# SEU-dynamical-models/Manifold-based-optical-flow-method

Measured on AMD Instinct MI355X. Metric: flow timesteps/sec on 160k-vertex mesh, higher is better.
Workload: dtype f32

## Files before the change

manifold-based-optical-flow-method_amd/csrc/mof_amg.hip:

```cpp
#include <algorithm>
#include <cstdio>
#include <cstdlib>

#include "mof_amg.h"
#include "mof_rowkern.h"

int mof_io_guard(const std::function<void()> &f);

namespace mof {

std::atomic<int> g_force_galerkin_ns{0};
enum GalKernel { kGal0Ns, kGal0Ent, kGalSys2F32, kGalSys2Bf16, kGalSys3, kGal3Ns, kGal3Ent, kGal3Big, kGalKernels };
std::atomic<int64_t> g_galerkin_launches[kGalKernels];

namespace {

constexpr int kB3 = 12;

__device__ __forceinline__ bool retired(const int32_t *sysi, int32_t b) {
    return !sysi[b * kSysStride + SI_ACTIVE] || sysi[b * kSysStride + SI_CONV] >= 0;
}

template <int BS>
__device__ __forceinline__ void ldv(const float *v, int64_t node, float (&x)[BS]) {
// ... 1063 lines not shown
        const int32_t i = F.rent[2 * (int64_t)e];
        const float *p = F.Q + (int64_t)F.rent[2 * (int64_t)e + 1] * (BSF * 3);
        float pm[BSF * 3];
#pragma unroll
        for (int k = 0; k < BSF * 3; ++k) pm[k] = p[k];
        float ri[kNSR][BSF];
#pragma unroll
        for (int t = 0; t < kNSR; ++t) ldr<BSF>(F.r, sm_b(F.sm, b0 + t), F.n, i, ri[t]);
#pragma unroll
        for (int t = 0; t < kNSR; ++t)
#pragma unroll
            for (int c = 0; c < 3; ++c) {
                float v = pm[c] * ri[t][0] + pm[3 + c] * ri[t][1];
                if constexpr (BSF == 3) v += pm[6 + c] * ri[t][2];
                c3[t][c] = v;
            }
    };
    for (int32_t q = e0 + threadIdx.x; q < e1 && !big; q += 2 * kWG) {
        const bool two = q + kWG < e1;
        const int32_t ea = F.rperm ? F.rperm[q] : q;
        const int32_t eb = two ? (F.rperm ? F.rperm[q + kWG] : q + kWG) : ea;
        float c3[2][kNSR][3];
        contrib(ea, c3[0]);
        contrib(eb, c3[1]);
#pragma unroll
        for (int t = 0; t < kNSR; ++t)
#pragma unroll
            for (int c = 0; c < 3; ++c) con[t][c][ea - e0] = c3[0][t][c];
        if (two)
#pragma unroll
            for (int t = 0; t < kNSR; ++t)
#pragma unroll
                for (int c = 0; c < 3; ++c) con[t][c][eb - e0] = c3[1][t][c];
    }
    __syncthreads();
    const int32_t nI = I1 - I0;
    for (int32_t q = threadIdx.x; q < nI * kNSR; q += kWG) {
        const int32_t t = q / nI, I = I0 + q - t * nI;
        if (b0 + t >= F.sm.n) continue;
        const int32_t b = sm_b(F.sm, b0 + t);
        if (retired(sysi, b)) continue;
        float acc[3] = {};
        for (int32_t e = F.rptr[I]; e < F.rptr[I + 1]; ++e) {
            float c3[3];
            if (big) {
                float all[kNSR][3];
                contrib(e, all);
#pragma unroll
                for (int c = 0; c < 3; ++c) c3[c] = all[t][c];
            } else {
#pragma unroll
                for (int c = 0; c < 3; ++c) c3[c] = con[t][c][e - e0];
            }
#pragma unroll
            for (int c = 0; c < 3; ++c) acc[c] += c3[c];
        }
        const int64_t vo = (int64_t)b * C.n * 4;
        stv<3>(C.b + vo, I, acc);
        if (smooth) {
            float d[3][3], x[3];
            ld_dh(C, b, I, d);
            matvec<3>(d, acc, x);
#pragma unroll
            for (int c = 0; c < 3; ++c) x[c] *= omega;
            stv<3>(C.x + vo, I, x);
        }
    }
}

template <int XM>
__global__ __launch_bounds__(kWG) void k_prolong0_sa(Lvl F, Lvl C, int32_t nblk, int32_t B,
                                                     const int32_t *__restrict__ sysi) {
#pragma clang fp contract(off)
    int32_t rb, bq;
    const int32_t nq = (F.sm.n + kNSP - 1) / kNSP;
    if (!xcd_map(nblk, nq, rb, bq, kGrpProl)) return;
    const int32_t b0 = bq * kNSP;
    const int32_t i = rb * kWG + threadIdx.x;
    if (i >= F.n) return;
    float x[kNSP][2];
#pragma unroll
    for (int t = 0; t < kNSP; ++t) {
        const float2 v = ld_x0(F.x, (int64_t)sm_b(F.sm, b0 + t) * F.n + i);
        x[t][0] = v.x;
        x[t][1] = v.y;
    }
    const int32_t k0 = F.pptr[i], k1 = F.pptr[i + 1];
    for (int32_t k = k0; k < k1; ++k) {
        const int32_t K = F.pcol[k];
        const float *q = F.Q + (int64_t)k * 6;
        float qm[6];
#pragma unroll
        for (int c = 0; c < 6; ++c) qm[c] = q[c];
        float y[kNSP][3];
#pragma unroll
        for (int t = 0; t < kNSP; ++t) ldv<3>(C.y + (int64_t)sm_b(F.sm, b0 + t) * C.n * 4, K, y[t]);
#pragma unroll
        for (int t = 0; t < kNSP; ++t) {
            x[t][0] += qm[0] * y[t][0] + qm[1] * y[t][1] + qm[2] * y[t][2];
            x[t][1] += qm[3] * y[t][0] + qm[4] * y[t][1] + qm[5] * y[t][2];
        }
    }
#pragma unroll
    for (int t = 0; t < kNSP; ++t) {
        if (b0 + t >= F.sm.n) continue;
        const int32_t b = sm_b(F.sm, b0 + t);
        if (retired(sysi, b)) continue;
        if constexpr (XM == 2)
            reinterpret_cast<float2 *>(F.y)[(int64_t)b * F.n + i] = make_float2(x[t][0], x[t][1]);
        else
            st_x0(F.x, (int64_t)b * F.n + i, x[t][0], x[t][1]);
    }
}

constexpr int kNS3 = 8;
__global__ __launch_bounds__(kWG) void k_prolong3_sa(Lvl F, Lvl C, int32_t nblk, int32_t B,
                                                     const int32_t *__restrict__ sysi) {
#pragma clang fp contract(off)
    int32_t rb, bq;
    if (!xcd_map(nblk, (F.sm.n + kNS3 - 1) / kNS3, rb, bq, kGrpProl)) return;
    const int32_t i = rb * kWG + threadIdx.x;
    if (i >= F.n) return;
    const int32_t b0 = bq * kNS3;
    float x[kNS3][3];
#pragma unroll
    for (int t = 0; t < kNS3; ++t) ldv<3>(F.x + (int64_t)sm_b(F.sm, b0 + t) * F.n * 4, i, x[t]);
    for (int32_t k = F.pptr[i]; k < F.pptr[i + 1]; ++k) {
        const float *p = F.Q + (int64_t)k * 9;
        float pm[9];
#pragma unroll
        for (int c = 0; c < 9; ++c) pm[c] = p[c];
        const int32_t K = F.pcol[k];
        float y[kNS3][3];
#pragma unroll
        for (int t = 0; t < kNS3; ++t) ldv<3>(C.y + (int64_t)sm_b(F.sm, b0 + t) * C.n * 4, K, y[t]);
#pragma unroll
        for (int t = 0; t < kNS3; ++t)
#pragma unroll
            for (int r = 0; r < 3; ++r) x[t][r] += pm[3 * r] * y[t][0] + pm[3 * r + 1] * y[t][1] + pm[3 * r + 2] * y[t][2];
    }
#pragma unroll
    for (int t = 0; t < kNS3; ++t) {
        if (b0 + t >= F.sm.n) continue;
        const int32_t b = sm_b(F.sm, b0 + t);
        if (retired(sysi, b)) continue;
        stv<3>(F.x + (int64_t)b * F.n * 4, i, x[t]);
    }
}

template <int BSF>
__global__ __launch_bounds__(kWG) void k_prolong(Lvl F, Lvl C, const int32_t *__restrict__ sysi) {
    const int32_t i = blockIdx.x * kWG + threadIdx.x, b = sm_b(F.sm, blockIdx.y);
    if (i >= F.n || retired(sysi, b)) return;
    prolong_node<BSF>(F, C, b, i);
}

constexpr int kProlR = 1, kProlS = 4;
template <int XM>
__global__ __launch_bounds__(kWG) void k_prolong0(Lvl F, Lvl C, int32_t nblk, int32_t B,
                                                  const int32_t *__restrict__ sysi) {
#pragma clang fp contract(off)
    int32_t rb, bq;
    if (!xcd_map(nblk, (F.sm.n + kProlS - 1) / kProlS, rb, bq, kGrpProl)) return;
    const int32_t n = F.n;
    int32_t ii[kProlR], ag[kProlR];
    float q[kProlR][6];
#pragma unroll
    for (int r = 0; r < kProlR; ++r) {
        ii[r] = (rb * kProlR + r) * kWG + threadIdx.x;
        const int32_t i = min(ii[r], n - 1);
        ag[r] = F.agg[i];
#pragma unroll
        for (int k = 0; k < 6; ++k) q[r][k] = F.Q[(int64_t)i * 6 + k];
    }
    float2 x0[kProlS][kProlR];
    float y[kProlS][kProlR][3];
#pragma unroll
    for (int t = 0; t < kProlS; ++t) {
        const int32_t b = sm_b(F.sm, bq * kProlS + t);
        const float *yb = C.y + (int64_t)b * C.n * 4;
#pragma unroll
        for (int r = 0; r < kProlR; ++r) {
            x0[t][r] = ld_x0(F.x, (int64_t)b * n + min(ii[r], n - 1));
            ldv<3>(yb, ag[r], y[t][r]);
        }
    }
#pragma unroll
    for (int t = 0; t < kProlS; ++t) {
        if (bq * kProlS + t >= F.sm.n) continue;
        const int32_t b = sm_b(F.sm, bq * kProlS + t);
        if (retired(sysi, b)) continue;
        const int64_t vb = (int64_t)b * n;
#pragma unroll
        for (int r = 0; r < kProlR; ++r) {
            if (ii[r] >= n) break;
            float xi[2] = {x0[t][r].x, x0[t][r].y};
#pragma unroll
            for (int k = 0; k < 2; ++k)
                xi[k] += q[r][3 * k] * y[t][r][0] + q[r][3 * k + 1] * y[t][r][1] + q[r][3 * k + 2] * y[t][r][2];
            if constexpr (XM == 2)
                reinterpret_cast<float2 *>(F.y)[vb + ii[r]] = make_float2(xi[0], xi[1]);
            else
                st_x0(F.x, vb + ii[r], xi[0], xi[1]);
        }
    }
}

__global__ __launch_bounds__(kWG) void k_post3(Lvl L, float omega, const int32_t *__restrict__ sysi) {
    const int32_t i = blockIdx.x * kWG + threadIdx.x, b = sm_b(L.sm, blockIdx.y);
    if (i >= L.n || retired(sysi, b)) return;
    post3_node(L, b, i, omega);
}

constexpr int kSubWG = 512;
constexpr int kMaxLevels = 12;

struct SubArgs {
    int32_t first, last;
    Lvl lv[kMaxLevels];
    const float *cinv;
    float omega;
    const int32_t *sysi;
};

__global__ __launch_bounds__(kSubWG) void k_subcycle(SubArgs a) {
    const int32_t b = sm_b(a.lv[0].sm, blockIdx.x);
    if (retired(a.sysi, b)) return;
    const int32_t tid = threadIdx.x;
    for (int32_t l = a.first; l < a.last; ++l) {
        const Lvl &F = a.lv[l], &C = a.lv[l + 1];
        for (int32_t i = tid; i < F.n; i += kSubWG) res3_node(F, b, i);
        __syncthreads();
        for (int32_t I = tid; I < C.n; I += kSubWG) restrict_node<3>(F, C, b, I, l + 1 < a.last, a.omega);
        __syncthreads();
    }
    {
        constexpr int kH = kSubWG / kMaxCoarse;
        __shared__ float bl[kMaxCoarse];
        __shared__ float part[kH][kMaxCoarse];
        const Lvl &C = a.lv[a.last];
        const int32_t nc = 3 * C.n;
        const float *Mi = a.cinv + (int64_t)b * nc * nc;
        const float *bb = C.b + (int64_t)b * C.n * 4;
        for (int32_t q = tid; q < nc; q += kSubWG) bl[q] = bb[4 * (q / 3) + q % 3];
        __syncthreads();
        const int32_t d = tid % kMaxCoarse, hf = tid / kMaxCoarse;
        const int32_t chunk = (nc + kH - 1) / kH;
        const int32_t k0 = min(nc, hf * chunk), k1 = min(nc, k0 + chunk);
        float sum = 0.f;
        if (d < nc) {
            constexpr int U = 16;
            for (int32_t k = k0; k < k1; k += U) {
                float mv[U];
#pragma unroll
                for (int u = 0; u < U; ++u) mv[u] = Mi[(int64_t)min(k + u, k1 - 1) * nc + d];
#pragma unroll
                for (int u = 0; u < U; ++u) sum += (k + u < k1) ? mv[u] * bl[min(k + u, k1 - 1)] : 0.f;
            }
        }
        part[hf][d] = sum;
        __syncthreads();
        if (!hf && d < nc) {
            float t = part[0][d];
#pragma unroll
            for (int h = 1; h < kH; ++h) t += part[h][d];
            C.y[(int64_t)b * C.n * 4 + 4 * (d / 3) + d % 3] = t;
        }
        __syncthreads();
    }
    for (int32_t l = a.last - 1; l >= a.first; --l) {
        const Lvl &F = a.lv[l], &C = a.lv[l + 1];
        for (int32_t i = tid; i < F.n; i += kSubWG) prolong_node<3>(F, C, b, i);
        __syncthreads();
        for (int32_t i = tid; i < F.n; i += kSubWG) post3_node(F, b, i, a.omega);
        __syncthreads();
    }
}

constexpr int kRes0NS = 2, kRes0U = kSweepU;
template <int NS, bool PK>
__global__ __launch_bounds__(kWG) MOF_ROW_OCC void k_res0_ns(int32_t N, int32_t nblk, int32_t B, SysMap sm, MatH mat,
                                                 const float *__restrict__ rv, const float *__restrict__ xv,
                                                 const int32_t *__restrict__ apos,
                                                 const int32_t *__restrict__ sysi, float *__restrict__ r1) {
#pragma clang fp contract(off)
    int32_t rb, bq;
    if (!xcd_map(nblk, (sm.n + NS - 1) / NS, rb, bq, kGrpSmooth > NS ? kGrpSmooth / NS : 1)) return;
    int32_t bs[NS];
    bool act[NS];
    bool any = false;
#pragma unroll
    for (int t = 0; t < NS; ++t) {
        const int32_t l = bq * NS + t;
        bs[t] = sm_b(sm, l);
        act[t] = l < sm.n && !retired(sysi, bs[t]);
        any |= act[t];
    }
    if (!any) return;
#pragma unroll
    for (int r = 0; r < kRows; ++r) {
        const int32_t i = rb * kRowsPerWG + r * kWG + threadIdx.x;
        if (i >= N) break;
        float y[NS][2];
        auto xl = [&](int t, int32_t j) { return ld_x0(xv, (int64_t)bs[t] * N + j); };
        if constexpr (PK)
            spmv_row_hx_ns<kIxPack, NS, kRes0U>(mat, bs, i, xl, y);
        else if (mat.sell_mir)
            spmv_row_hx_ns<kIxMir, NS, kRes0U>(mat, bs, i, xl, y);
        else
            spmv_row_hx_ns<kIxPlain, NS, kRes0U>(mat, bs, i, xl, y);
#pragma unroll
        for (int t = 0; t < NS; ++t) {
            if (!act[t]) continue;
            const int64_t vb = (int64_t)bs[t] * N;
            const float2 ri = reinterpret_cast<const float2 *>(rv)[vb + i];
            reinterpret_cast<uint32_t *>(r1)[vb + (apos ? apos[i] : i)] =
                bf16_bits(ri.x - y[t][0]) | (bf16_bits(ri.y - y[t][1]) << 16);
        }
    }
}

constexpr int kPost0NS = 2, kPost0U = 4;
template <int XM, bool ZH, int NS, bool PK>
__global__ __launch_bounds__(kWG) MOF_ROW_OCC void k_post0_ns(int32_t N, int32_t nblk, int32_t B, SysMap sm, MatH mat,
                                                  const float *__restrict__ rv,
                                                  const float *__restrict__ xv, float omega,
                                                  const int32_t *__restrict__ sysi,
                                                  float *__restrict__ zv, double *__restrict__ part,
                                                  RedArgs rd) {
#pragma clang fp contract(off)
    __shared__ double lds[8 * NS];
    int32_t rb, bq;
    if (!xcd_map(nblk, (sm.n + NS - 1) / NS, rb, bq, kGrpSmooth > NS ? kGrpSmooth / NS : 1)) return;
    int32_t bs[NS];
    bool act[NS];
    bool any = false;
#pragma unroll
    for (int t = 0; t < NS; ++t) {
        const int32_t l = bq * NS + t;
        bs[t] = sm_b(sm, l);
        act[t] = l < sm.n && !retired(sysi, bs[t]);
        any |= act[t];
    }
    if (!any) return;
    double rz[NS];
#pragma unroll
    for (int t = 0; t < NS; ++t) rz[t] = 0.0;
#pragma unroll
    for (int g = 0; g < kRows; ++g) {
        const int32_t i = rb * kRowsPerWG + g * kWG + threadIdx.x;
        if (i >= N) break;
        float y[NS][2];
        uint2 dg[NS];
        auto xl = [&](int t, int32_t j) {
            const int64_t vj = (int64_t)bs[t] * N + j;
            if constexpr (XM == 2)
                return reinterpret_cast<const float2 *>(xv)[vj];
            else
                return ld_x0(xv, vj);
        };
        if constexpr (PK)
            spmv_row_hx_ns<kIxPack, NS, kPost0U>(mat, bs, i, xl, y, dg);
        else if (mat.sell_mir)
            spmv_row_hx_ns<kIxMir, NS, kPost0U>(mat, bs, i, xl, y, dg);
        else
            spmv_row_hx_ns<kIxPlain, NS, kPost0U>(mat, bs, i, xl, y, dg);
#pragma unroll
        for (int t = 0; t < NS; ++t) {
            const int64_t vb = (int64_t)bs[t] * N;
            const float2 xi = xl(t, i);
            const float2 ri = reinterpret_cast<const float2 *>(rv)[vb + i];
            const float2 ds = bf16_diag_solve(dg[t], ri.x - y[t][0], ri.y - y[t][1]);
            float z0 = xi.x + omega * ds.x;
            float z1 = xi.y + omega * ds.y;
            if constexpr (ZH) {
                const uint32_t h = bf16_bits(z0) | (bf16_bits(z1) << 16);
                if (act[t]) reinterpret_cast<uint32_t *>(zv)[vb + i] = h;
                z0 = bf16_lo(h);
                z1 = bf16_hi(h);
            } else {
                if (act[t]) reinterpret_cast<float2 *>(zv)[vb + i] = make_float2(z0, z1);
            }
            if (i < rd.nown) rz[t] += (double)ri.x * z0 + (double)ri.y * z1;
        }
    }
    block_sum<NS>(rz, lds);
    if (threadIdx.x == 0) {
#pragma unroll
        for (int t = 0; t < NS; ++t)
            if (act[t]) part[2 * (((int64_t)rd.part * B + bs[t]) * rd.nmax + rb)] = rz[t];
    }
}

constexpr int kBswWG = 1024;
constexpr int32_t kBswOff = INT32_MIN;
constexpr int64_t kBswLdsMax = 160 * 1024;
struct BswArgs {
    int32_t N, nbr, nout, nslot;
    const int32_t *rows, *roff, *wrow, *xsrc, *ocol;
    const uint2 *A;
};
template <bool F32X>
__device__ __forceinline__ float2 bsw_ldx(const float *xv, int64_t vj) {
    if constexpr (F32X)
        return reinterpret_cast<const float2 *>(xv)[vj];
    else
        return ld_x0(xv, vj);
}
__global__ __launch_bounds__(kWG) void k_bsw_extract(int32_t nslot, int32_t B, const int32_t *__restrict__ bsrc,
                                                     const uint2 *__restrict__ A0h, int64_t sell_nb,
                                                     uint2 *__restrict__ out) {
    const int64_t q = (int64_t)blockIdx.x * kWG + threadIdx.x;
    if (q >= (int64_t)nslot * B) return;
    const int32_t b = (int32_t)(q / nslot), t = (int32_t)(q - (int64_t)b * nslot);
    const int32_t src = bsrc[t];
    uint2 h = make_uint2(0u, 0u);
    if (src >= 0) {
        h = h0_ld(A0h, (int64_t)b * sell_nb + (src & kMirPos));
        if (src & kMirT) h = h0_tr(h);
    }
    out[q] = h;
}
template <bool F32X>
__global__ __launch_bounds__(kBswWG) void k_bsweep(BswArgs a, SysMap sm, const float *__restrict__ rv,
                                                   float *__restrict__ xv, float omega, int32_t sweeps,
                                                   const int32_t *__restrict__ sysi) {
#pragma clang fp contract(off)
    extern __shared__ float2 bsw_lds[];
    if ((int32_t)blockIdx.x >= sm.n) return;
    const int32_t b = sm_b(sm, blockIdx.x);
    if (retired(sysi, b)) return;
    const int64_t vb = (int64_t)b * a.N;
    float2 *xs[2] = {bsw_lds, bsw_lds + a.nbr};
    float2 *xo = bsw_lds + 2 * a.nbr;
    for (int32_t p = threadIdx.x; p < a.nbr; p += kBswWG) xs[0][p] = bsw_ldx<F32X>(xv, vb + a.rows[p]);
    for (int32_t k = threadIdx.x; k < a.nout; k += kBswWG) xo[k] = bsw_ldx<F32X>(xv, vb + a.ocol[k]);
    __syncthreads();
    const uint2 *Ab = a.A + (int64_t)b * a.nslot;
    constexpr int U = kPost0U;
    int cur = 0;
    for (int32_t k = 0; k < sweeps; ++k) {
        for (int32_t p = threadIdx.x; p < a.nbr; p += kBswWG) {
            const int32_t base = a.roff[p >> 6] + (p & 63), w = a.wrow[p];
            const float2 ri = reinterpret_cast<const float2 *>(rv)[vb + a.rows[p]];
            float acc0 = 0.f, acc1 = 0.f;
            uint2 dg = make_uint2(0u, 0u);
            for (int32_t t0 = 0; t0 < w; t0 += U) {
                int32_t src[U];
                uint2 blk[U];
#pragma unroll
                for (int u = 0; u < U; ++u) {
                    const int32_t q = base + min(t0 + u, w - 1) * kSlice;
                    src[u] = a.xsrc[q];
                    blk[u] = Ab[q];
                }
                if (t0 == 0) dg = blk[0];
#pragma unroll
                for (int u = 0; u < U; ++u) {
                    const bool on = t0 + u < w && src[u] != kBswOff;
                    float2 xj = make_float2(0.f, 0.f);
                    if (on) xj = src[u] >= 0 ? xs[cur][src[u]] : xo[-1 - src[u]];
                    float e00, e01, e10, e11;
                    h0_dec(blk[u], e00, e01, e10, e11);
                    acc0 += on ? e00 * xj.x + e01 * xj.y : 0.f;
                    acc1 += on ? e10 * xj.x + e11 * xj.y : 0.f;
                }
            }
            const float2 ds = bf16_diag_solve(dg, ri.x - acc0, ri.y - acc1);
            const float2 xi = xs[cur][p];
            xs[cur ^ 1][p] = make_float2(xi.x + omega * ds.x, xi.y + omega * ds.y);
        }
        __syncthreads();
        cur ^= 1;
    }
    for (int32_t p = threadIdx.x; p < a.nbr; p += kBswWG) {
        const float2 v = xs[cur][p];
        if constexpr (F32X)
            reinterpret_cast<float2 *>(xv)[vb + a.rows[p]] = v;
        else
            st_x0(xv, vb + a.rows[p], v.x, v.y);
    }
}
BswArgs bsw_args(const AmgDevice &G) {
    BswArgs a;
    a.N = G.bsw_N;
    a.nbr = G.bsw_n;
    a.nout = G.bsw_nout;
    a.nslot = G.bsw_nslot;
    a.rows = G.bsw_rows.p;
    a.roff = G.bsw_roff.p;
    a.wrow = G.bsw_wrow.p;
    a.xsrc = G.bsw_xsrc.p;
    a.ocol = G.bsw_ocol.p;
    a.A = reinterpret_cast<const uint2 *>(G.bsw_A.p);
    return a;
}
template <bool F32X>
void launch_bsweep(const AmgDevice &G, SysMap sm, const float *rv, float *xv, float omega, const int32_t *sysi,
                   hipStream_t s) {
    const size_t lds = sizeof(float2) * (2 * (size_t)G.bsw_n + G.bsw_nout);
    k_bsweep<F32X><<<dim3((unsigned)sm.n), kBswWG, lds, s>>>(bsw_args(G), sm, rv, xv, omega, G.bsw_sweeps, sysi);
}

template <int XM, bool ZH, typename... Args>
void launch_post0(bool packed, int32_t nblk, int32_t B, hipStream_t s, Args... args) {
    const dim3 g(xcd_grid(nblk, (B + kPost0NS - 1) / kPost0NS, kGrpSmooth > kPost0NS ? kGrpSmooth / kPost0NS : 1));
    if (packed)
        k_post0_ns<XM, ZH, kPost0NS, true><<<g, kWG, 0, s>>>(args...);
    else
        k_post0_ns<XM, ZH, kPost0NS, false><<<g, kWG, 0, s>>>(args...);
}

inline dim3 grid2(int64_t n, int32_t B) { return dim3((unsigned)((n + kWG - 1) / kWG), (unsigned)B); }

MatH level0_mat(mof_mesh *m) {
    MatH mt;
    mt.sell_nb = m->pat.sell_nb();
    mt.sell_off = m->sell_off.p;
    mt.sell_col = m->sell_col.p;
    mt.sell_mir = m->sym_reads ? m->sell_mir.p : nullptr;
    mt.sell_idx = m->sym_reads && m->idx_packed ? m->sell_idx.p : nullptr;
    mt.vptr = m->sym_reads ? nullptr : m->vptr.p;
    mt.A = reinterpret_cast<const uint2 *>(m->amg->A0h.p);
    return mt;
}

}


bool amg_build(mof_mesh *m) {
    AmgParams prm;
    const bool open_surface = [&] {
        const int64_t E = ((int64_t)m->pat.nblocks() - m->N) / 2;
        return m->n_own == m->N && 3 * (int64_t)m->M != 2 * E;
    }();
    if (open_surface) {
        prm.omega = 0.7f;
        prm.smooth = 1;
    }
    float omega1_set = 0.f;
    if (const char *v = knob(Knob::AmgOmega)) {
        char *end = nullptr;
        prm.omega = std::strtof(v, &end);
        if (end && *end == ',') omega1_set = prm.omega1 = std::strtof(end + 1, nullptr);
    }
    if (knob(Knob::AmgSmooth)) prm.smooth = knob_int(Knob::AmgSmooth, 0) != 0;
    prm.smooth1 = -1;
    if (m->n_own < m->N) prm.nown = m->n_own;
    if (m->amg && m->amg->built) return m->amg->lv.size() >= 2;
    if (!m->amg) m->amg = new AmgDevice();
    AmgDevice &G = *m->amg;
    hipStream_t s = m->stream;
    MeshShared *sh = m->shared.get();
    char key[160];
    std::snprintf(key, sizeof(key), "%a/%a/%d/%d/%a/%d/%d", (double)prm.omega, (double)prm.omega1, prm.smooth,
                  prm.nown, (double)prm.smooth_omega, (int)m->sym_reads, prm.smooth1);
    std::unique_lock<std::mutex> build_lock;
    std::shared_ptr<const AmgHierarchy> Hp;
    if (sh) {
        build_lock = std::unique_lock<std::mutex>(sh->amg_build_mu);
        std::lock_guard<std::mutex> lk(sh->mu);
        for (const auto &kv : sh->amg)
            if (kv.first == key) Hp = kv.second;
    }
    if (!Hp) {
        std::vector<double> e(6 * (size_t)m->N);
        MOF_HIP(hipMemcpyAsync(e.data(), m->e.p, e.size() * sizeof(double), hipMemcpyDeviceToHost, s));
        MOF_HIP(hipStreamSynchronize(s));
        std::vector<double> a2;
        if (prm.nown < 0 && ((prm.smooth != 0 && (prm.smooth > 0 || amg_auto_smooth(m->pat))) || prm.smooth1 != 0)) {
            a2.resize(4 * (size_t)m->pat.sell_nb());
            MOF_HIP(hipMemcpyAsync(a2.data(), m->a2.p, a2.size() * sizeof(double), hipMemcpyDeviceToHost, s));
            MOF_HIP(hipStreamSynchronize(s));
            prm.a2 = a2.data();
        }
        if (!m->agg_order.empty()) prm.order = m->agg_order.data();
        const std::vector<int32_t> mir = sell_mirror(m->pat, m->n_own, 1, nullptr);
        prm.mirror = mir.data();
        auto built = std::make_shared<AmgHierarchy>();
        AmgParams p1 = prm;
        const bool l0_smooth = prm.nown < 0 && prm.a2 && prm.smooth != 0 && (prm.smooth > 0 || amg_auto_smooth(m->pat));
        p1.smooth1 = prm.smooth1 > 0 ? prm.smooth1 : (prm.smooth1 < 0 && l0_smooth ? 1 : 0);
        if (open_surface && p1.smooth1 == 1) p1.smooth1 = 2;
        build_amg(m->pat, e.data(), p1, *built);
        if (prm.smooth1 < 0 && p1.smooth1 == 0 && prm.nown < 0 && prm.a2 && !built->levels.empty() &&
            !built->levels[0].smoothed && built->max_curl >= kFoldCurl) {
            const double curl = built->max_curl;
            p1.smooth1 = 1;
            if (prm.smooth != 0 && !built->curl.empty() && built->curl[0] < kFlatCurl) p1.smooth = 1;
            auto again = std::make_shared<AmgHierarchy>();
            build_amg(m->pat, e.data(), p1, *again);
            again->max_curl = curl;
            again->folded = true;
            built = again;
        }
        built->mirror = mir;
        Hp = built;
        if (sh) {
            std::lock_guard<std::mutex> lk(sh->mu);
            sh->amg.emplace_back(key, Hp);
        }
    }
    if (build_lock.owns_lock()) build_lock.unlock();
    const AmgHierarchy &H = *Hp;
    G.H = Hp;
    G.omega = prm.omega;
    G.omega1 = prm.omega1;
    G.xm = 2;
    G.lv.clear();
    G.built = true;
    if (H.levels.size() < 2) return false;
    G.regular = !amg_auto_smooth(m->pat) && !open_surface;
    G.xm = G.regular ? 1 : 2;
    if (omega1_set <= 0.f) G.omega1 = G.regular ? 1.1f : 1.05f;
    MOF_REQUIRE(H.coarse_dofs <= kMaxCoarse, "coarsest multigrid level too large");
    MOF_REQUIRE(H.levels.size() <= (size_t)kMaxLevels, "too many multigrid levels");
    G.lv.resize(H.levels.size());
    auto put_i = [&](DevArray<int32_t> &d, const std::vector<int32_t> &h) {
        d.alloc(h.size());
        if (!h.empty()) d.upload(h.data(), h.size(), s);
    };
    auto put_f = [&](DevArray<float> &d, const std::vector<float> &h) {
        d.alloc(h.size());
        if (!h.empty()) d.upload(h.data(), h.size(), s);
    };
    G.bsw_n = 0;
    G.bsw_sweeps = 0;
    int32_t bsw = -1;
    if (knob(Knob::AmgBsw)) bsw = std::max(0, std::min(8, knob_int(Knob::AmgBsw, 0)));
    if (open_surface && bsw != 0) {
        const Pattern &P = m->pat;
        std::vector<uint8_t> mark(m->N, 0);
        for (int32_t i = 0; i < m->N; ++i) {
            const int32_t a = P.vptr[i], e2 = P.vptr[i + 1];
            const int32_t d = (int32_t)(std::lower_bound(P.vcol.begin() + a, P.vcol.begin() + e2, i) - P.vcol.begin());
            if (P.cptr[d + 1] - P.cptr[d] < e2 - a - 1) mark[i] = 1;
        }
        std::vector<uint8_t> ring(mark);
        for (int32_t i = 0; i < m->N; ++i)
            if (mark[i])
                for (int32_t q = P.vptr[i]; q < P.vptr[i + 1]; ++q) ring[P.vcol[q]] = 1;
        std::vector<int32_t> rows, pos(m->N, -1);
        for (int32_t i = 0; i < m->N; ++i)
            if (ring[i]) {
                pos[i] = (int32_t)rows.size();
                rows.push_back(i);
            }
        if (!rows.empty()) {
            const int32_t nbr = (int32_t)rows.size(), nrs = (nbr + kSlice - 1) / kSlice;
            std::vector<int32_t> mir;
            if (m->sym_reads) mir = sell_mirror(P, m->n_own, 1, nullptr);
            std::vector<int32_t> wrow(nbr), roff(nrs + 1, 0), ocol, opos(m->N, -1);
            for (int32_t p = 0; p < nbr; ++p) {
                const int32_t s0 = rows[p] / kSlice;
                wrow[p] = (int32_t)((P.sell_off[s0 + 1] - P.sell_off[s0]) / kSlice);
            }
            for (int32_t r = 0; r < nrs; ++r) {
                int32_t wmax = 0;
                for (int32_t p = r * kSlice; p < std::min(nbr, (r + 1) * kSlice); ++p) wmax = std::max(wmax, wrow[p]);
                roff[r + 1] = roff[r] + wmax * kSlice;
            }
            const int32_t nslot = roff[nrs];
            std::vector<int32_t> xsrc(nslot, kBswOff), bsrc(nslot, -1);
            for (int32_t p = 0; p < nbr; ++p) {
                const int32_t i = rows[p], s0 = i / kSlice, l = i % kSlice;
                const int64_t o = P.sell_off[s0];
                const int32_t w = wrow[p];
                const int32_t wl = m->sym_reads ? w : std::min(w, P.vptr[i + 1] - P.vptr[i]);
                for (int32_t t = 0; t < w; ++t) {
                    const int64_t pp = o + (int64_t)std::min(t, wl - 1) * kSlice + l;
                    const int32_t j = P.sell_col[pp];
                    int32_t src = (int32_t)pp;
                    bool on = t < wl;
                    if (m->sym_reads) {
                        const int32_t mr = mir[pp];
                        on = on && mr >= 0;
                        src = mr < 0 ? (int32_t)(o + l) : mr;
                    }
                    if (!on) continue;
                    const int64_t q = roff[p / kSlice] + (int64_t)t * kSlice + p % kSlice;
                    bsrc[q] = src;
                    if (pos[j] >= 0) {
                        xsrc[q] = pos[j];
                    } else {
                        if (opos[j] < 0) {
                            opos[j] = (int32_t)ocol.size();
                            ocol.push_back(j);
                        }
                        xsrc[q] = -1 - opos[j];
                    }
                }
            }
            const int64_t lds = (int64_t)sizeof(float2) * (2 * (int64_t)nbr + (int64_t)ocol.size());
            if (lds > kBswLdsMax) {
                if (knob(Knob::Verbose))
                    std::fprintf(stderr, "mof amg: boundary ring of %d rows needs %lld B of LDS: no boundary sweeps\n",
                                 nbr, (long long)lds);
            } else {
                put_i(G.bsw_rows, rows);
                put_i(G.bsw_roff, roff);
                put_i(G.bsw_wrow, wrow);
                put_i(G.bsw_xsrc, xsrc);
                put_i(G.bsw_bsrc, bsrc);
                put_i(G.bsw_ocol, ocol);
                G.bsw_N = m->N;
                G.bsw_n = nbr;
                G.bsw_nout = (int32_t)ocol.size();
                G.bsw_nslot = nslot;
                G.bsw_sweeps = bsw > 0 ? bsw : 2;
                if (knob(Knob::Verbose))
                    std::fprintf(stderr, "mof amg: boundary sweeps x%d on a ring of %d rows (%d outside, %lld B of LDS)\n",
                                 G.bsw_sweeps, nbr, G.bsw_nout, (long long)lds);
                static LdsLimit limit;
                raise_lds_limit(limit, m->device,
                                {reinterpret_cast<const void *>(&k_bsweep<true>),
                                 reinterpret_cast<const void *>(&k_bsweep<false>)},
                                kBswLdsMax);
            }
        }
    }
    for (size_t l = 0; l < H.levels.size(); ++l) {
        const AmgLevel &L = H.levels[l];
        AmgDevLevel &D = G.lv[l];
        D.n = L.n;
        D.bs = L.bs;
        D.sell_nb = L.sell_nb();
        if (l > 0) {
            {
                std::vector<int32_t> tw((size_t)L.sell_nb(), -1);
                for (size_t k = 0; k < L.low.size(); ++k) tw[L.twin[k]] = L.low[k];
                put_i(D.twin, tw);
            }
            put_i(D.sell_off, L.sell_off);
            put_i(D.sell_col, L.sell_col);
            put_i(D.sell_row, L.sell_row);
            put_i(D.diag_pos, L.diag_pos);
            D.dead.alloc(L.dead.size());
            D.dead.upload(L.dead.data(), L.dead.size(), s);
        }
        if (l + 1 < H.levels.size()) {
            put_i(D.agg, L.agg);
            put_i(D.mptr, L.mptr);
// ... 529 lines not shown
```

manifold-based-optical-flow-method_amd/csrc/mof_rowkern.h:

```cpp
#pragma once

#include "mof_internal.h"

namespace mof {
namespace {

template <typename V>
struct VT;
template <>
struct VT<float> {
    using V2 = float2;
};
template <>
struct VT<double> {
    using V2 = double2;
};

constexpr int kRows = 1;
constexpr int kRowsPerWG = kWG * kRows;

__device__ __forceinline__ void ld_blk(const float *A, int64_t pos, float (&a)[4]) {
    const float4 v = reinterpret_cast<const float4 *>(A)[pos];
    a[0] = v.x; a[1] = v.y; a[2] = v.z; a[3] = v.w;
}
__device__ __forceinline__ void ld_blk(const double *A, int64_t pos, double (&a)[4]) {
    const double2 v0 = reinterpret_cast<const double2 *>(A)[2 * pos];
    const double2 v1 = reinterpret_cast<const double2 *>(A)[2 * pos + 1];
    a[0] = v0.x; a[1] = v0.y; a[2] = v1.x; a[3] = v1.y;
}

__device__ __forceinline__ uint32_t bf16_bits(float f) {
    const uint32_t u = __float_as_uint(f);
    return (u + 0x7FFFu + ((u >> 16) & 1u)) >> 16;
}
__device__ __forceinline__ float bf16_lo(uint32_t w) { return __uint_as_float(w << 16); }
__device__ __forceinline__ float bf16_hi(uint32_t w) { return __uint_as_float(w & 0xFFFF0000u); }
__device__ __forceinline__ uint2 bf16x4(float a, float b, float c, float d) {
    return make_uint2(bf16_bits(a) | (bf16_bits(b) << 16), bf16_bits(c) | (bf16_bits(d) << 16));
}

__device__ __forceinline__ uint2 h0_ld(const uint2 *H, int64_t q) { return H[q]; }
__device__ __forceinline__ void h0_st(uint2 *H, int64_t q, float a, float b, float c, float d) {
    H[q] = bf16x4(a, b, c, d);
}
__device__ __forceinline__ uint2 h0_tr(uint2 h) {
    return make_uint2((h.x & 0xFFFFu) | (h.y << 16), (h.x >> 16) | (h.y & 0xFFFF0000u));
}
__device__ __forceinline__ void h0_dec(uint2 h, float &a00, float &a01, float &a10, float &a11) {
    a00 = bf16_lo(h.x); a01 = bf16_hi(h.x); a10 = bf16_lo(h.y); a11 = bf16_hi(h.y);
}

__device__ __forceinline__ double wave_sum(double v) {
#pragma unroll
    for (int o = 32; o > 0; o >>= 1) v += __shfl_down(v, o, 64);
    return v;
}

template <int NV, int NT = kWG>
__device__ __forceinline__ void block_sum(double (&v)[NV], double *lds) {
#pragma unroll
    for (int k = 0; k < NV; ++k) v[k] = wave_sum(v[k]);
    const int w = threadIdx.x >> 6;
    if ((threadIdx.x & 63) == 0) {
#pragma unroll
        for (int k = 0; k < NV; ++k) lds[w * NV + k] = v[k];
    }
    __syncthreads();
#pragma unroll
    for (int k = 0; k < NV; ++k) {
        double s = ((lds[k] + lds[NV + k]) + lds[2 * NV + k]) + lds[3 * NV + k];
#pragma unroll
        for (int q = 4; q < NT / 64; ++q) s += lds[q * NV + k];
        v[k] = s;
    }
    __syncthreads();
}

template <int NV, int NQ>
__device__ __forceinline__ void block_sum_q(double (&v)[NV], double *lds) {
    if constexpr (NQ == 1) {
        block_sum<NV, kWG>(v, lds);
    } else {
#pragma unroll
        for (int k = 0; k < NV; ++k) v[k] = wave_sum(v[k]);
        const int w = threadIdx.x >> 6;
        if ((threadIdx.x & 63) == 0) {
#pragma unroll
            for (int k = 0; k < NV; ++k) lds[w * NV + k] = v[k];
        }
        __syncthreads();
        const double *L = lds + (w & ~3) * NV;
#pragma unroll
        for (int k = 0; k < NV; ++k) v[k] = ((L[k] + L[NV + k]) + L[2 * NV + k]) + L[3 * NV + k];
        __syncthreads();
    }
}
__device__ __forceinline__ int32_t row_tid() { return (int32_t)(threadIdx.x & (kWG - 1)); }

__device__ __forceinline__ double wave_max(double v) {
#pragma unroll
    for (int o = 32; o > 0; o >>= 1) v = fmax(v, __shfl_down(v, o, 64));
    return v;
}
template <int NV, int NQ>
__device__ __forceinline__ void block_max_q(double (&v)[NV], double *lds) {
#pragma unroll
    for (int k = 0; k < NV; ++k) v[k] = wave_max(v[k]);
    const int w = threadIdx.x >> 6;
    if ((threadIdx.x & 63) == 0) {
#pragma unroll
        for (int k = 0; k < NV; ++k) lds[w * NV + k] = v[k];
    }
    __syncthreads();
    const double *L = lds + (w & ~3) * NV;
#pragma unroll
    for (int k = 0; k < NV; ++k) v[k] = fmax(fmax(L[k], L[NV + k]), fmax(L[2 * NV + k], L[3 * NV + k]));
    __syncthreads();
}
template <int NV, int NT>
__device__ __forceinline__ void block_max(double (&v)[NV], double *lds) {
#pragma unroll
    for (int k = 0; k < NV; ++k) v[k] = wave_max(v[k]);
    const int w = threadIdx.x >> 6;
    if ((threadIdx.x & 63) == 0) {
#pragma unroll
        for (int k = 0; k < NV; ++k) lds[w * NV + k] = v[k];
    }
    __syncthreads();
#pragma unroll
    for (int k = 0; k < NV; ++k) {
        double s = lds[k];
#pragma unroll
        for (int q = 1; q < NT / 64; ++q) s = fmax(s, lds[q * NV + k]);
        v[k] = s;
    }
    __syncthreads();
}

template <int NV, int NT = kWG>
__device__ __forceinline__ void reduce_partials(const double *part, int n, double (&out)[NV],
                                                double *lds) {
#pragma unroll
    for (int k = 0; k < NV; ++k) out[k] = 0.0;
    int q = threadIdx.x < kWG ? (int)threadIdx.x : n;
    for (; q + 3 * kWG < n; q += 4 * kWG) {
        double v[4][NV];
#pragma unroll
        for (int u = 0; u < 4; ++u)
#pragma unroll
            for (int k = 0; k < NV; ++k) v[u][k] = part[(int64_t)(q + u * kWG) * NV + k];
#pragma unroll
        for (int u = 0; u < 4; ++u)
#pragma unroll
            for (int k = 0; k < NV; ++k) out[k] += v[u][k];
    }
    for (; q < n; q += kWG) {
#pragma unroll
        for (int k = 0; k < NV; ++k) out[k] += part[(int64_t)q * NV + k];
    }
    block_sum<NV, NT>(out, lds);
}

template <typename V>
struct MatArgs {
    int64_t sell_nb;
    const int32_t *sell_off, *sell_col;
    const int32_t *sell_mir;
    const uint32_t *sell_idx;
    const int32_t *vptr;
    const V *A;
};

__device__ __forceinline__ int32_t row_width(const int32_t *vptr, int32_t i, int32_t w) {
    return vptr ? min(w, vptr[i + 1] - vptr[i]) : w;
}

__device__ __forceinline__ int64_t mir_pos(int32_t m, int64_t diag) { return m < 0 ? diag : (int64_t)(m & kMirPos); }

template <typename V>
__device__ __forceinline__ typename VT<V>::V2 ld2(const V *p) {
    return *reinterpret_cast<const typename VT<V>::V2 *>(p);
}

constexpr int kIxPlain = 0, kIxMir = 1, kIxPack = 2;
__device__ __forceinline__ int32_t idx_dcol(uint32_t w) { return (int32_t)(w << 16) >> 16; }
__device__ __forceinline__ int32_t idx_dpos(uint32_t w) { return (int32_t)w >> 16; }

__device__ __forceinline__ int32_t wave_slice(int32_t i) { return __builtin_amdgcn_readfirstlane(i >> 6); }

template <typename T>
__device__ __forceinline__ const T *byte_off(const T *base, uint32_t bytes) {
    return reinterpret_cast<const T *>(reinterpret_cast<const char *>(base) + bytes);
}
__device__ __forceinline__ void ld_blk32(const float *A, uint32_t pos, float (&a)[4]) {
    const float4 v = *byte_off(reinterpret_cast<const float4 *>(A), pos * 16u);
    a[0] = v.x; a[1] = v.y; a[2] = v.z; a[3] = v.w;
}
__device__ __forceinline__ void ld_blk32(const double *A, uint32_t pos, double (&a)[4]) { ld_blk(A, (int64_t)pos, a); }

#define MOF_ROW_OCC __attribute__((amdgpu_waves_per_eu(5, 8)))
constexpr int kSpmvU = 8, kSweepU = 8;

template <int IX, typename V, bool ZH = false>
__device__ __forceinline__ void spmv_row_t(const MatArgs<V> &mt, int32_t b, int32_t i,
                                           const V *__restrict__ x, V &y0, V &y1) {
#pragma clang fp contract(off)
    using V2 = typename VT<V>::V2;
    constexpr int U = kSpmvU;
    constexpr bool sym = IX != kIxPlain;
    const V *A = mt.A + 4 * (int64_t)b * mt.sell_nb;
    const int32_t s = wave_slice(i), l = i & 63;
    const int32_t o = mt.sell_off[s];
    const int32_t w = (mt.sell_off[s + 1] - o) >> 6;
    const int32_t wl = sym ? w : row_width(mt.vptr, i, w);
    V a0 = 0, a1 = 0;
    for (int32_t t0 = 0; t0 < w; t0 += U) {
        int32_t j[U], mr[U];
        V blk[U][4];
        V2 xj[U];
#pragma unroll
        for (int u = 0; u < U; ++u) {
            const int32_t t = min(t0 + u, wl - 1);
            if constexpr (IX == kIxPack) {
                const uint32_t iw = *byte_off(mt.sell_idx, (uint32_t)(o + t * kSlice + l) * 4u);
                j[u] = i + idx_dcol(iw);
                mr[u] = idx_dpos(iw);
            } else {
                j[u] = mt.sell_col[(int64_t)o + t * kSlice + l];
                if constexpr (sym) mr[u] = mt.sell_mir[(int64_t)o + t * kSlice + l];
            }
        }
#pragma unroll
        for (int u = 0; u < U; ++u) {
            const int32_t t = min(t0 + u, wl - 1);
            if constexpr (IX == kIxPack)
                ld_blk32(A, (uint32_t)(mr[u] == kIdxPad ? o + l : o + t * kSlice + l + mr[u]), blk[u]);
            else if constexpr (sym)
                ld_blk(A, mir_pos(mr[u], (int64_t)o + l), blk[u]);
            else
                ld_blk(A, (int64_t)o + t * kSlice + l, blk[u]);
        }
#pragma unroll
        for (int u = 0; u < U; ++u) {
            if constexpr (ZH) {
                const uint32_t h = reinterpret_cast<const uint32_t *>(x)[j[u]];
                xj[u] = V2{bf16_lo(h), bf16_hi(h)};
            } else {
                xj[u] = ld2(x + 2 * (int64_t)j[u]);
            }
        }
#pragma unroll
        for (int u = 0; u < U; ++u) {
            if constexpr (sym) {
                bool on, tr;
                if constexpr (IX == kIxPack) {
                    on = t0 + u < w && mr[u] != kIdxPad;
                    tr = mr[u] != 0;
                } else {
                    on = t0 + u < w && mr[u] >= 0;
                    tr = (mr[u] & kMirT) != 0;
                }
                const V b1 = tr ? blk[u][2] : blk[u][1], b2 = tr ? blk[u][1] : blk[u][2];
                a0 += on ? blk[u][0] * xj[u].x + b1 * xj[u].y : (V)0;
                a1 += on ? b2 * xj[u].x + blk[u][3] * xj[u].y : (V)0;
            } else {
                const bool on = t0 + u < wl;
                a0 += on ? blk[u][0] * xj[u].x + blk[u][1] * xj[u].y : (V)0;
                a1 += on ? blk[u][2] * xj[u].x + blk[u][3] * xj[u].y : (V)0;
            }
        }
    }
    y0 = a0;
    y1 = a1;
}
template <typename V, bool ZH = false>
__device__ __forceinline__ void spmv_row(const MatArgs<V> &mt, int32_t b, int32_t i,
                                         const V *__restrict__ x, V &y0, V &y1) {
    if (mt.sell_mir)
        spmv_row_t<kIxMir, V, ZH>(mt, b, i, x, y0, y1);
    else
        spmv_row_t<kIxPlain, V, ZH>(mt, b, i, x, y0, y1);
}

constexpr int32_t kGrpSpmv = 8, kGrpSmooth = 8, kGrpRes = 8, kGrpGal = 8, kGrpAsm = 8, kGrpProl = 8,
                  kGrpRestr = 8;
__host__ __device__ __forceinline__ int32_t sys_group(int32_t B, int32_t G) { return G > 0 && G < B ? G : B; }

__host__ __device__ __forceinline__ bool xcd_map_w(int32_t w, int32_t nblk, int32_t B, int32_t &rb, int32_t &sys,
                                                   int32_t grp_sz) {
    const int32_t q = w >> 3;
    const int32_t chunk = (nblk + 7) >> 3;
    const int32_t G = sys_group(B, grp_sz);
    const int32_t grp = q / (chunk * G), rem = q - grp * chunk * G;
    sys = grp * G + rem % G;
    rb = (w & 7) * chunk + rem / G;
    return rb < nblk && sys < B;
}
__device__ __forceinline__ bool xcd_map(int32_t nblk, int32_t B, int32_t &rb, int32_t &sys, int32_t grp_sz) {
    return xcd_map_w((int32_t)blockIdx.x, nblk, B, rb, sys, grp_sz);
}

inline unsigned xcd_grid(int32_t nblk, int32_t B, int32_t grp_sz) {
    const int64_t G = sys_group(B, grp_sz);
    const int64_t n = 8 * G * ((B + G - 1) / G) * ((nblk + 7) / 8);
    MOF_REQUIRE(n * kWG < ((int64_t)1 << 32), "launch grid past 2^32 work-items (batch too large for this mesh)");
    return (unsigned)n;
}
inline int32_t xcd_batch_cap(int64_t nblk, int32_t grp_sz) {
    const int64_t lim = (((int64_t)1 << 32) - 1) / kWG;
    const int64_t per = 8 * ((nblk + 7) / 8);
    int64_t B = std::min<int64_t>(lim / per, 1 << 30);
    auto n = [&](int64_t b) {
        const int64_t G = b > grp_sz && grp_sz > 0 ? grp_sz : b;
        return 8 * G * ((b + G - 1) / G) * ((nblk + 7) / 8);
    };
    while (B > 1 && n(B) > lim) --B;
    return (int32_t)std::max<int64_t>(1, B);
}


struct SysMap {
    const int32_t *map;
    int32_t n;
};
inline SysMap sys_all(int32_t B) { return SysMap{nullptr, B}; }
__device__ __forceinline__ int32_t sm_b(const SysMap &s, int32_t l) {
    l = min(l, s.n - 1);
    return s.map ? s.map[l] : l;
}

struct MatH {
    int64_t sell_nb;
    const int32_t *sell_off, *sell_col;
    const int32_t *sell_mir;
    const uint32_t *sell_idx;
    const int32_t *vptr;
    const uint2 *A;
};

template <int IX, int NS, int U = kSweepU, typename XL>
__device__ __forceinline__ void spmv_row_hx_ns(const MatH &mt, const int32_t (&bs)[NS], int32_t i, XL &&xload,
                                               float (&y)[NS][2], uint2 *diag = nullptr) {
#pragma clang fp contract(off)
    constexpr bool sym = IX != kIxPlain;
    using Pos = std::conditional_t<IX == kIxPack, uint32_t, int64_t>;
    const int32_t s = wave_slice(i), l = i & 63;
    const int32_t o = mt.sell_off[s];
    const int32_t w = (mt.sell_off[s + 1] - o) >> 6;
    const int32_t wl = sym ? w : row_width(mt.vptr, i, w);
    float acc[NS][2];
#pragma unroll
    for (int t = 0; t < NS; ++t) acc[t][0] = acc[t][1] = 0.f;
    for (int32_t t0 = 0; t0 < w; t0 += U) {
        int32_t j[U], mr[U];
        Pos pos[U];
#pragma unroll
        for (int u = 0; u < U; ++u) {
            if constexpr (IX == kIxPack) {
                const int32_t own = o + min(t0 + u, wl - 1) * kSlice + l;
                const uint32_t iw = *byte_off(mt.sell_idx, (uint32_t)own * 4u);
                j[u] = i + idx_dcol(iw);
                mr[u] = idx_dpos(iw);
                pos[u] = (uint32_t)(mr[u] == kIdxPad ? o + l : own + mr[u]);
            } else {
                pos[u] = (int64_t)o + min(t0 + u, wl - 1) * kSlice + l;
                j[u] = mt.sell_col[pos[u]];
                if constexpr (sym) mr[u] = mt.sell_mir[pos[u]];
            }
        }
        if constexpr (IX == kIxMir) {
#pragma unroll
            for (int u = 0; u < U; ++u) pos[u] = mir_pos(mr[u], (int64_t)o + l);
        }
        uint2 blk[NS][U];
        float2 xj[NS][U];
#pragma unroll
        for (int t = 0; t < NS; ++t) {
            if constexpr (IX == kIxPack) {
                const uint2 *Ab = mt.A + (int64_t)bs[t] * mt.sell_nb;
#pragma unroll
                for (int u = 0; u < U; ++u) blk[t][u] = *byte_off(Ab, pos[u] * 8u);
            } else {
#pragma unroll
                for (int u = 0; u < U; ++u) blk[t][u] = h0_ld(mt.A, (int64_t)bs[t] * mt.sell_nb + pos[u]);
            }
        }
        if (diag && t0 == 0) {
#pragma unroll
            for (int t = 0; t < NS; ++t) diag[t] = blk[t][0];
        }
#pragma unroll
        for (int t = 0; t < NS; ++t)
#pragma unroll
            for (int u = 0; u < U; ++u) xj[t][u] = xload(t, j[u]);
#pragma unroll
        for (int u = 0; u < U; ++u) {
            bool on = t0 + u < wl;
            bool tr = false;
            if constexpr (IX == kIxPack) {
                on = on && mr[u] != kIdxPad;
                tr = mr[u] != 0;
            } else if constexpr (sym) {
                on = on && mr[u] >= 0;
                tr = (mr[u] & kMirT) != 0;
            }
#pragma unroll
            for (int t = 0; t < NS; ++t) {
                const uint2 h = tr ? h0_tr(blk[t][u]) : blk[t][u];
                float e00, e01, e10, e11;
                h0_dec(h, e00, e01, e10, e11);
                acc[t][0] += on ? e00 * xj[t][u].x + e01 * xj[t][u].y : 0.f;
                acc[t][1] += on ? e10 * xj[t][u].x + e11 * xj[t][u].y : 0.f;
            }
        }
    }
#pragma unroll
    for (int t = 0; t < NS; ++t) {
        y[t][0] = acc[t][0];
        y[t][1] = acc[t][1];
    }
}

__device__ __forceinline__ float2 ld_x0(const float *x, int64_t vi) {
    const uint32_t h = reinterpret_cast<const uint32_t *>(x)[vi];
    return make_float2(bf16_lo(h), bf16_hi(h));
}
__device__ __forceinline__ void st_x0(float *x, int64_t vi, float a, float b) {
    reinterpret_cast<uint32_t *>(x)[vi] = bf16_bits(a) | (bf16_bits(b) << 16);
}

__device__ __forceinline__ float2 bf16_mat2(uint2 d, float v0, float v1) {
    return make_float2(bf16_lo(d.x) * v0 + bf16_hi(d.x) * v1, bf16_lo(d.y) * v0 + bf16_hi(d.y) * v1);
}

__device__ __forceinline__ float2 bf16_diag_solve(uint2 a, float v0, float v1) {
    float a00, a01, a10, a11;
    h0_dec(a, a00, a01, a10, a11);
    const float id = 1.f / (a00 * a11 - a01 * a10);
    return make_float2((a11 * v0 - a01 * v1) * id, (a00 * v1 - a10 * v0) * id);
}
__device__ __forceinline__ uint2 bf16_diag_block(const uint2 *A, int64_t sell_nb, const int32_t *sell_off,
                                                 int32_t b, int32_t i) {
    return h0_ld(A, (int64_t)b * sell_nb + sell_off[wave_slice(i)] + (i & 63));
}

}
}
```

Baseline: 4373.

## Restructure SELL row SpMV inner loops with exact-width batches and packed math

Row SpMV kernels now process full unrolled batches and then dispatch a compile-time-sized tail batch, so symmetric and f32 paths skip padded slots instead of clamping and masking them. The multi-system kernel accumulates with 2-wide vector floats and defers bf16 decoding of x until use. Packed-index paths use 32-bit byte offsets for x loads. The post-smoother unroll rises from 4 to 7 while the block sweep keeps 4. Scheduling barriers are inserted per element. The aim is less wasted work on padding and better memory-level parallelism, at the cost of more code and register pressure, and the barriers may restrict instruction scheduling.

```diff
diff --git a/manifold-based-optical-flow-method_amd/csrc/mof_amg.hip b/manifold-based-optical-flow-method_amd/csrc/mof_amg.hip
--- a/manifold-based-optical-flow-method_amd/csrc/mof_amg.hip
+++ b/manifold-based-optical-flow-method_amd/csrc/mof_amg.hip
@@ -1389,7 +1389,12 @@
         const int32_t i = rb * kRowsPerWG + r * kWG + threadIdx.x;
         if (i >= N) break;
         float y[NS][2];
-        auto xl = [&](int t, int32_t j) { return ld_x0(xv, (int64_t)bs[t] * N + j); };
+        auto xl = [&](int t, int32_t j) {
+            if constexpr (PK)
+                return ld_x0w_32(xv + (int64_t)bs[t] * N, j);
+            else
+                return ld_x0w(xv, (int64_t)bs[t] * N + j);
+        };
         if constexpr (PK)
             spmv_row_hx_ns<kIxPack, NS, kRes0U>(mat, bs, i, xl, y);
         else if (mat.sell_mir)
@@ -1407,7 +1412,7 @@
     }
 }
 
-constexpr int kPost0NS = 2, kPost0U = 4;
+constexpr int kPost0NS = 2, kPost0U = 7;
 template <int XM, bool ZH, int NS, bool PK>
 __global__ __launch_bounds__(kWG) MOF_ROW_OCC void k_post0_ns(int32_t N, int32_t nblk, int32_t B, SysMap sm, MatH mat,
                                                   const float *__restrict__ rv,
@@ -1441,10 +1446,14 @@
         uint2 dg[NS];
         auto xl = [&](int t, int32_t j) {
             const int64_t vj = (int64_t)bs[t] * N + j;
-            if constexpr (XM == 2)
+            if constexpr (PK && XM == 2)
+                return ld_f2_32(xv + 2 * (int64_t)bs[t] * N, j);
+            else if constexpr (PK)
+                return ld_x0w_32(xv + (int64_t)bs[t] * N, j);
+            else if constexpr (XM == 2)
                 return reinterpret_cast<const float2 *>(xv)[vj];
             else
-                return ld_x0(xv, vj);
+                return ld_x0w(xv, vj);
         };
         if constexpr (PK)
             spmv_row_hx_ns<kIxPack, NS, kPost0U>(mat, bs, i, xl, y, dg);
@@ -1455,7 +1464,7 @@
 #pragma unroll
         for (int t = 0; t < NS; ++t) {
             const int64_t vb = (int64_t)bs[t] * N;
-            const float2 xi = xl(t, i);
+            const f32x2 xi = x_pair(xl(t, i));
             const float2 ri = reinterpret_cast<const float2 *>(rv)[vb + i];
             const float2 ds = bf16_diag_solve(dg[t], ri.x - y[t][0], ri.y - y[t][1]);
             float z0 = xi.x + omega * ds.x;
@@ -1524,7 +1533,7 @@
     for (int32_t k = threadIdx.x; k < a.nout; k += kBswWG) xo[k] = bsw_ldx<F32X>(xv, vb + a.ocol[k]);
     __syncthreads();
     const uint2 *Ab = a.A + (int64_t)b * a.nslot;
-    constexpr int U = kPost0U;
+    constexpr int U = 4;
     int cur = 0;
     for (int32_t k = 0; k < sweeps; ++k) {
         for (int32_t p = threadIdx.x; p < a.nbr; p += kBswWG) {
diff --git a/manifold-based-optical-flow-method_amd/csrc/mof_rowkern.h b/manifold-based-optical-flow-method_amd/csrc/mof_rowkern.h
--- a/manifold-based-optical-flow-method_amd/csrc/mof_rowkern.h
+++ b/manifold-based-optical-flow-method_amd/csrc/mof_rowkern.h
@@ -201,6 +201,18 @@
 #define MOF_ROW_OCC __attribute__((amdgpu_waves_per_eu(5, 8)))
 constexpr int kSpmvU = 8, kSweepU = 8;
 
+template <int K>
+using KC = std::integral_constant<int, K>;
+template <int K, typename F>
+__device__ __forceinline__ void tail_batch(int32_t r, F &&f) {
+    if constexpr (K > 0) {
+        if (r == K)
+            f(KC<K>{});
+        else
+            tail_batch<K - 1>(r, f);
+    }
+}
+
 template <int IX, typename V, bool ZH = false>
 __device__ __forceinline__ void spmv_row_t(const MatArgs<V> &mt, int32_t b, int32_t i,
                                            const V *__restrict__ x, V &y0, V &y1) {
@@ -208,19 +220,23 @@
     using V2 = typename VT<V>::V2;
     constexpr int U = kSpmvU;
     constexpr bool sym = IX != kIxPlain;
+    constexpr bool exact = !std::is_same_v<V, double>;
     const V *A = mt.A + 4 * (int64_t)b * mt.sell_nb;
     const int32_t s = wave_slice(i), l = i & 63;
     const int32_t o = mt.sell_off[s];
     const int32_t w = (mt.sell_off[s + 1] - o) >> 6;
     const int32_t wl = sym ? w : row_width(mt.vptr, i, w);
     V a0 = 0, a1 = 0;
-    for (int32_t t0 = 0; t0 < w; t0 += U) {
-        int32_t j[U], mr[U];
-        V blk[U][4];
-        V2 xj[U];
-#pragma unroll
-        for (int u = 0; u < U; ++u) {
-            const int32_t t = min(t0 + u, wl - 1);
+    auto batch = [&](int32_t t0, auto kc, auto padc) {
+#pragma clang fp contract(off)
+        constexpr int K = decltype(kc)::value;
+        constexpr bool PAD = decltype(padc)::value;
+        int32_t j[K], mr[K];
+        V blk[K][4];
+        std::conditional_t<ZH, uint32_t, V2> xr[K];
+#pragma unroll
+        for (int u = 0; u < K; ++u) {
+            const int32_t t = PAD || !sym ? min(t0 + u, wl - 1) : t0 + u;
             if constexpr (IX == kIxPack) {
                 const uint32_t iw = *byte_off(mt.sell_idx, (uint32_t)(o + t * kSlice + l) * 4u);
                 j[u] = i + idx_dcol(iw);
@@ -231,8 +247,8 @@
             }
         }
 #pragma unroll
-        for (int u = 0; u < U; ++u) {
-            const int32_t t = min(t0 + u, wl - 1);
+        for (int u = 0; u < K; ++u) {
+            const int32_t t = PAD || !sym ? min(t0 + u, wl - 1) : t0 + u;
             if constexpr (IX == kIxPack)
                 ld_blk32(A, (uint32_t)(mr[u] == kIdxPad ? o + l : o + t * kSlice + l + mr[u]), blk[u]);
             else if constexpr (sym)
@@ -241,34 +257,53 @@
                 ld_blk(A, (int64_t)o + t * kSlice + l, blk[u]);
         }
 #pragma unroll
-        for (int u = 0; u < U; ++u) {
-            if constexpr (ZH) {
-                const uint32_t h = reinterpret_cast<const uint32_t *>(x)[j[u]];
-                xj[u] = V2{bf16_lo(h), bf16_hi(h)};
-            } else {
-                xj[u] = ld2(x + 2 * (int64_t)j[u]);
-            }
-        }
-#pragma unroll
-        for (int u = 0; u < U; ++u) {
+        for (int u = 0; u < K; ++u) {
+            if constexpr (ZH && IX == kIxPack)
+                xr[u] = *byte_off(reinterpret_cast<const uint32_t *>(x), (uint32_t)j[u] * 4u);
+            else if constexpr (ZH)
+                xr[u] = reinterpret_cast<const uint32_t *>(x)[j[u]];
+            else if constexpr (IX == kIxPack)
+                xr[u] = *byte_off(reinterpret_cast<const V2 *>(x), (uint32_t)j[u] * (uint32_t)sizeof(V2));
+            else
+                xr[u] = ld2(x + 2 * (int64_t)j[u]);
+        }
+#pragma unroll
+        for (int u = 0; u < K; ++u) {
+            if constexpr (!PAD) __builtin_amdgcn_sched_barrier(0);
+            V2 xv;
+            if constexpr (ZH)
+                xv = V2{bf16_lo(xr[u]), bf16_hi(xr[u])};
+            else
+                xv = xr[u];
+            const bool in = !PAD || t0 + u < w;
             if constexpr (sym) {
                 bool on, tr;
                 if constexpr (IX == kIxPack) {
-                    on = t0 + u < w && mr[u] != kIdxPad;
+                    on = in && mr[u] != kIdxPad;
                     tr = mr[u] != 0;
                 } else {
-                    on = t0 + u < w && mr[u] >= 0;
+                    on = in && mr[u] >= 0;
                     tr = (mr[u] & kMirT) != 0;
                 }
                 const V b1 = tr ? blk[u][2] : blk[u][1], b2 = tr ? blk[u][1] : blk[u][2];
-                a0 += on ? blk[u][0] * xj[u].x + b1 * xj[u].y : (V)0;
-                a1 += on ? b2 * xj[u].x + blk[u][3] * xj[u].y : (V)0;
+                const V p0 = blk[u][0] * xv.x + b1 * xv.y, p1 = b2 * xv.x + blk[u][3] * xv.y;
+                a0 += on ? p0 : (V)0;
+                a1 += on ? p1 : (V)0;
             } else {
                 const bool on = t0 + u < wl;
-                a0 += on ? blk[u][0] * xj[u].x + blk[u][1] * xj[u].y : (V)0;
-                a1 += on ? blk[u][2] * xj[u].x + blk[u][3] * xj[u].y : (V)0;
+                const V p0 = blk[u][0] * xv.x + blk[u][1] * xv.y;
+                const V p1 = blk[u][2] * xv.x + blk[u][3] * xv.y;
+                a0 += on ? p0 : (V)0;
+                a1 += on ? p1 : (V)0;
             }
         }
+    };
+    if constexpr (exact) {
+        int32_t t0 = 0;
+        for (; t0 + U <= w; t0 += U) batch(t0, KC<U>{}, std::false_type{});
+        tail_batch<U - 1>(w - t0, [&](auto kc) { batch(t0, kc, std::false_type{}); });
+    } else {
+        for (int32_t t0 = 0; t0 < w; t0 += U) batch(t0, KC<U>{}, std::true_type{});
     }
     y0 = a0;
     y1 = a1;
@@ -329,6 +364,11 @@
     return s.map ? s.map[l] : l;
 }
 
+typedef float f32x2 __attribute__((ext_vector_type(2)));
+
+__device__ __forceinline__ f32x2 x_pair(uint32_t h) { return f32x2{bf16_lo(h), bf16_hi(h)}; }
+__device__ __forceinline__ f32x2 x_pair(float2 v) { return f32x2{v.x, v.y}; }
+
 struct MatH {
     int64_t sell_nb;
     const int32_t *sell_off, *sell_col;
@@ -348,41 +388,43 @@
     const int32_t o = mt.sell_off[s];
     const int32_t w = (mt.sell_off[s + 1] - o) >> 6;
     const int32_t wl = sym ? w : row_width(mt.vptr, i, w);
-    float acc[NS][2];
-#pragma unroll
-    for (int t = 0; t < NS; ++t) acc[t][0] = acc[t][1] = 0.f;
-    for (int32_t t0 = 0; t0 < w; t0 += U) {
-        int32_t j[U], mr[U];
-        Pos pos[U];
-#pragma unroll
-        for (int u = 0; u < U; ++u) {
+    f32x2 acc[NS];
+#pragma unroll
+    for (int t = 0; t < NS; ++t) acc[t] = f32x2{0.f, 0.f};
+    auto batch = [&](int32_t t0, auto kc) {
+#pragma clang fp contract(off)
+        constexpr int K = decltype(kc)::value;
+        int32_t j[K], mr[K];
+        Pos pos[K];
+#pragma unroll
+        for (int u = 0; u < K; ++u) {
             if constexpr (IX == kIxPack) {
-                const int32_t own = o + min(t0 + u, wl - 1) * kSlice + l;
+                const int32_t own = o + (sym ? t0 + u : min(t0 + u, wl - 1)) * kSlice + l;
                 const uint32_t iw = *byte_off(mt.sell_idx, (uint32_t)own * 4u);
                 j[u] = i + idx_dcol(iw);
                 mr[u] = idx_dpos(iw);
                 pos[u] = (uint32_t)(mr[u] == kIdxPad ? o + l : own + mr[u]);
             } else {
-                pos[u] = (int64_t)o + min(t0 + u, wl - 1) * kSlice + l;
+                pos[u] = (int64_t)o + (sym ? t0 + u : min(t0 + u, wl - 1)) * kSlice + l;
                 j[u] = mt.sell_col[pos[u]];
                 if constexpr (sym) mr[u] = mt.sell_mir[pos[u]];
             }
         }
         if constexpr (IX == kIxMir) {
 #pragma unroll
-            for (int u = 0; u < U; ++u) pos[u] = mir_pos(mr[u], (int64_t)o + l);
-        }
-        uint2 blk[NS][U];
-        float2 xj[NS][U];
+            for (int u = 0; u < K; ++u) pos[u] = mir_pos(mr[u], (int64_t)o + l);
+        }
+        uint2 blk[NS][K];
+        decltype(xload(0, 0)) xj[NS][K];
 #pragma unroll
         for (int t = 0; t < NS; ++t) {
             if constexpr (IX == kIxPack) {
                 const uint2 *Ab = mt.A + (int64_t)bs[t] * mt.sell_nb;
 #pragma unroll
-                for (int u = 0; u < U; ++u) blk[t][u] = *byte_off(Ab, pos[u] * 8u);
+                for (int u = 0; u < K; ++u) blk[t][u] = *byte_off(Ab, pos[u] * 8u);
             } else {
 #pragma unroll
-                for (int u = 0; u < U; ++u) blk[t][u] = h0_ld(mt.A, (int64_t)bs[t] * mt.sell_nb + pos[u]);
+                for (int u = 0; u < K; ++u) blk[t][u] = h0_ld(mt.A, (int64_t)bs[t] * mt.sell_nb + pos[u]);
             }
         }
         if (diag && t0 == 0) {
@@ -392,10 +434,11 @@
 #pragma unroll
         for (int t = 0; t < NS; ++t)
 #pragma unroll
-            for (int u = 0; u < U; ++u) xj[t][u] = xload(t, j[u]);
-#pragma unroll
-        for (int u = 0; u < U; ++u) {
-            bool on = t0 + u < wl;
+            for (int u = 0; u < K; ++u) xj[t][u] = xload(t, j[u]);
+#pragma unroll
+        for (int u = 0; u < K; ++u) {
+            __builtin_amdgcn_sched_barrier(0);
+            bool on = sym || t0 + u < wl;
             bool tr = false;
             if constexpr (IX == kIxPack) {
                 on = on && mr[u] != kIdxPad;
@@ -406,24 +449,37 @@
             }
 #pragma unroll
             for (int t = 0; t < NS; ++t) {
-                const uint2 h = tr ? h0_tr(blk[t][u]) : blk[t][u];
                 float e00, e01, e10, e11;
-                h0_dec(h, e00, e01, e10, e11);
-                acc[t][0] += on ? e00 * xj[t][u].x + e01 * xj[t][u].y : 0.f;
-                acc[t][1] += on ? e10 * xj[t][u].x + e11 * xj[t][u].y : 0.f;
+                h0_dec(blk[t][u], e00, e01, e10, e11);
+                const f32x2 cd = {e00, e11}, co = {tr ? e10 : e01, tr ? e01 : e10};
+                const f32x2 xv = x_pair(xj[t][u]);
+                const f32x2 p = cd * xv + co * xv.yx;
+                acc[t] += on ? p : f32x2{0.f, 0.f};
             }
         }
-    }
+    };
+    int32_t t0 = 0;
+    for (; t0 + U <= w; t0 += U) batch(t0, KC<U>{});
+    tail_batch<U - 1>(w - t0, [&](auto kc) { batch(t0, kc); });
 #pragma unroll
     for (int t = 0; t < NS; ++t) {
-        y[t][0] = acc[t][0];
-        y[t][1] = acc[t][1];
+        y[t][0] = acc[t].x;
+        y[t][1] = acc[t].y;
     }
 }
 
 __device__ __forceinline__ float2 ld_x0(const float *x, int64_t vi) {
     const uint32_t h = reinterpret_cast<const uint32_t *>(x)[vi];
     return make_float2(bf16_lo(h), bf16_hi(h));
+}
+__device__ __forceinline__ uint32_t ld_x0w(const float *x, int64_t vi) {
+    return reinterpret_cast<const uint32_t *>(x)[vi];
+}
+__device__ __forceinline__ uint32_t ld_x0w_32(const float *xb, int32_t j) {
+    return *byte_off(reinterpret_cast<const uint32_t *>(xb), (uint32_t)j * 4u);
+}
+__device__ __forceinline__ float2 ld_f2_32(const float *xb, int32_t j) {
+    return *byte_off(reinterpret_cast<const float2 *>(xb), (uint32_t)j * 8u);
 }
 __device__ __forceinline__ void st_x0(float *x, int64_t vi, float a, float b) {
     reinterpret_cast<uint32_t *>(x)[vi] = bf16_bits(a) | (bf16_bits(b) << 16);
```

After: 4410, median of 3. About the same (+0.9%).
